# 1dayac/spades_for_blackbird

Hardware: AMD Instinct MI355X
Metric: distinct k-mers/sec (k=21, 150 bp synthetic reads, count only) (higher is better)
Workload: dtype u64

## Files before the change

### spades_for_blackbird_amd/csrc/bbk_internal.h

```cpp
#pragma once

#include <hip/hip_runtime.h>

#include <cstdint>
#include <cstdio>
#include <cstdlib>
#include <map>
#include <memory>
#include <string>
#include <type_traits>
#include <utility>
#include <vector>

#include "../../include/bbk.h"

namespace bbk {

void set_error(const char *fmt, ...);

struct Error {
    int code;
};

#define BBK_HIP(expr)                                                                          \
// ... 226 lines not shown
struct PassDesc {
    int kind;
    int word;
    int shift;
    int bits;
    unsigned nb;
};

std::vector<PassDesc> key_passes(unsigned k);

void sort_records(bbk_ctx *ctx, int W, void *keys, void *keys_tmp, uint32_t *vals, uint32_t *vals_tmp, uint64_t n,
                  const std::vector<PassDesc> &passes);
void partition_records(bbk_ctx *ctx, int W, const void *src, void *dst, const uint32_t *vsrc, uint32_t *vdst, uint64_t n,
                       const PassDesc &pd, uint64_t *h_digit_totals = nullptr);

enum ReduceOp { REDUCE_COUNT = 0, REDUCE_SUM = 1, REDUCE_OR = 2 };
uint64_t unique_records(bbk_ctx *ctx, int W, const void *keys, const uint32_t *vals, uint64_t n, void *out_keys,
                        uint32_t *out_vals, ReduceOp op, bool drop_zero);
uint64_t drop_zero_vals(bbk_ctx *ctx, int W, const void *keys, const uint32_t *vals, uint64_t n, DevBuf &out_keys,
                        DevBuf &out_vals);
uint64_t exclusive_scan_u64(bbk_ctx *ctx, const uint64_t *in, uint64_t *out, uint64_t n);
void exclusive_scan2_u64(bbk_ctx *ctx, const uint64_t *in0, uint64_t *out0, const uint64_t *in1, uint64_t *out1,
                         uint64_t n, uint64_t totals[2]);
enum { SCAN_U64 = 0, SCAN_U32_FLAGGED = 1, SCAN_SLOT_FILL = 2 };
struct ScanSrc {
    const void *p;
    uint32_t kind, stride, cap;
};
void exclusive_scan_enqueue(bbk_ctx *ctx, int narr, const ScanSrc *src, uint64_t *const *out, uint64_t n,
                            uint64_t *d_total, bool tail, std::vector<DevBuf> &keep);
struct PrefixTable;
struct PrefixIndex {
    DevBuf buf;
    unsigned bits = 0;
    bool wide = false;
    unsigned W = 0, k = 0;
    void build(bbk_ctx *ctx, const uint64_t *keys, unsigned W, unsigned k, uint64_t n);
    PrefixTable table() const;
};
size_t device_free_cached(bbk_ctx *ctx);
void *plan_staging(bbk_ctx *ctx, size_t bytes);

}

extern "C" int bbk_scan2_u64(bbk_ctx *ctx, void *d_a, void *d_b, uint64_t n, uint64_t *totals);

struct bbk_reads {
    bbk_ctx *ctx = nullptr;
    uint64_t n = 0;
    uint64_t n_words = 0;
    uint64_t bases = 0;
    const uint64_t *d_words = nullptr;
    const uint64_t *d_woff = nullptr;
    const uint32_t *d_len = nullptr;
    bbk::DevBuf own_words, own_woff, own_len;
};

struct bbk_kmerset {
    unsigned k = 0, W = 0;
    unsigned flags = 0;
    uint64_t n = 0;
    uint64_t instances = 0;
    bbk::DevBuf keys;
    bbk::DevBuf counts;
    bool has_counts = false;
    bool sorted = true;
    bool ref_order = false;
};

struct bbk_extindex {
    unsigned k = 0, W = 0;
    uint64_t n = 0;
    uint64_t instances = 0;
    bbk::DevBuf keys;
    bbk::DevBuf masks;
    bbk::PrefixIndex prefix;
};
```

### spades_for_blackbird_amd/csrc/count.hip

```cpp
#include <hip/hip_runtime.h>

#include <fcntl.h>
#include <unistd.h>

#include <algorithm>
#include <cstdio>
#include <cstring>
#include <memory>
#include <vector>

#include "bbk_internal.h"
#include "kmer_ops.h"
#include "msd.h"
#include "accum.h"

namespace bbk {

static bool msd_enabled() {
    const char *e = getenv("BBK_DISABLE_MSD");
    return !(e && e[0] == '1');
}

__global__ void k_kmers_per_read(const uint32_t *__restrict__ len, uint64_t n, uint32_t k,
                                 uint64_t *__restrict__ nk) {
    const uint64_t i = BBK_GID();
    if (i < n) {
        const uint32_t L = len[i];
        nk[i] = L >= k ? (uint64_t)(L - k + 1) : 0ull;
    }
}

template <int W, int MODE>
__global__ __launch_bounds__(256) void k_extract(const uint64_t *__restrict__ words,
                                                const uint64_t *__restrict__ woff,
                                                const uint32_t *__restrict__ len,
                                                const uint64_t *__restrict__ koff, uint64_t n_reads, int k,
                                                Key<W> *__restrict__ out, uint32_t *__restrict__ out_val) {
    const int lane = threadIdx.x & 63;
    const uint64_t wave = (BBK_GID()) >> 6;
    const uint64_t nwaves = ((uint64_t)gridDim.x * blockDim.x) >> 6;
    for (uint64_t r = wave; r < n_reads; r += nwaves) {
        const uint32_t L = len[r];
        if (L < (uint32_t)k) continue;
        const uint32_t nk = L - (uint32_t)k + 1;
        const uint64_t *rw = words + woff[r];
        const uint64_t base = koff[r];
        for (uint32_t p = lane; p < nk; p += 64) {
            const Key<W> fwd = kmer_extract<W>(rw, p, k);
            const Key<W> rc = kmer_rc<W>(fwd, k);
            const bool minimal = !kmer_less_nucl<W>(rc, fwd);
            out[base + p] = key_select<W>(minimal, fwd, rc);
            if (MODE == 1) {
// ... 125 lines not shown
    }
};

void dedup_reads(bbk_ctx *ctx, const bbk_reads *rd, unsigned k, bool with_mask, bool want_vals, DevBuf &out_keys,
                 DevBuf &out_vals, uint64_t &n_distinct, uint64_t &n_instances, BucketView *view = nullptr) {
    n_distinct = 0;
    n_instances = 0;
    if (msd_enabled()) {
        const int op1 = with_mask ? MSD_OP_OR : (want_vals ? MSD_OP_COUNT : MSD_OP_NONE);
        if (superk_dedup_reads(ctx, rd, k, op1, out_keys, out_vals, n_distinct, n_instances)) return;
        n_distinct = 0;
        n_instances = 0;
        MsdOutput a;
        a.want_view = view != nullptr;
        if (msd_sort_reduce(ctx, k, MsdRequest::reads(MSD_HASH, op1, rd, with_mask), a)) {
            n_instances = a.instances;
            n_distinct = a.n;
            if (a.view.live()) *view = std::move(a.view);
            out_keys = std::move(a.keys);
            if (op1 != MSD_OP_NONE) out_vals = std::move(a.vals);
            return;
        }
    }
    DevBuf koff((rd->n + 1) * sizeof(uint64_t));
    if (rd->n) launch_items(ctx, "k_kmers_per_read", k_kmers_per_read, rd->n, rd->d_len, rd->n, k, koff.as<uint64_t>());
    const uint64_t N = exclusive_scan_u64(ctx, koff.as<uint64_t>(), koff.as<uint64_t>(), rd->n);
    n_instances = N;
    if (N == 0) return empty_result(out_keys, &out_vals);
    BBK_REQUIRE(N < (1ull << 32), BBK_ERR_ARG,
                "batch holds %llu k-mer instances; the LSD path is limited to 2^32-1 per batch (push the reads in "
                "smaller batches)",
                (unsigned long long)N);
    LsdSort t(ctx, k, N, with_mask);
    dispatch_w(t.W, [&](auto w) {
        launch_extract<decltype(w)::value>(ctx, rd, koff.as<uint64_t>(), (int)k, t.keys.p, t.vals.as<uint32_t>(), N);
    });
    t.sort();
    n_distinct =
        t.unique(with_mask ? REDUCE_OR : REDUCE_COUNT, out_keys, (with_mask || want_vals) ? &out_vals : nullptr);
}

static uint64_t lsd_sort_unique(bbk_ctx *ctx, unsigned k, const void *d_keys, const uint32_t *d_vals, uint64_t n,
                                ReduceOp rop, DevBuf &out_keys, DevBuf &out_vals) {
    LsdSort t(ctx, k, n, d_vals != nullptr);
    t.load(d_keys, d_vals);
    t.sort();
    return t.unique(rop, out_keys, d_vals ? &out_vals : nullptr);
}

// ... 562 lines not shown
```

### spades_for_blackbird_amd/csrc/kmer_ops.h

```cpp
#pragma once

#include <hip/hip_runtime.h>
#include <stdint.h>

namespace bbk {

template <int W>
struct Key {
    uint64_t w[W];
};

template <int W>
__host__ __device__ inline bool key_eq(const Key<W> &a, const Key<W> &b) {
    bool e = true;
#pragma unroll
    for (int i = 0; i < W; ++i) e = e && (a.w[i] == b.w[i]);
    return e;
}

template <int W>
__host__ __device__ inline bool key_less_words(const Key<W> &a, const Key<W> &b) {
#pragma unroll
    for (int i = 0; i < W; ++i) {
        if (a.w[i] != b.w[i]) return a.w[i] < b.w[i];
// ... 118 lines not shown
        if (a.w[i] != b.w[i]) return rev2(a.w[i]) < rev2(b.w[i]);
    }
    return false;
}

template <int W>
__device__ inline Key<W> kmer_canon(const uint64_t *__restrict__ rw, uint32_t p, int k, uint32_t last_word, bool *minimal) {
    if constexpr (W == 1) {
        return kmer_extract_canon1(rw, p, k, last_word, minimal);
    } else {
        const Key<W> x = kmer_extract<W>(rw, p, k);
        const Key<W> r = kmer_rc<W>(x, k);
        *minimal = !kmer_less_nucl<W>(r, x);
        return key_select<W>(*minimal, x, r);
    }
}

__device__ inline uint64_t last_le(const uint64_t *__restrict__ off, uint64_t n, uint64_t x) {
    uint64_t lo = 0, hi = n - 1;
    while (lo < hi) {
        const uint64_t mid = (lo + hi + 1) >> 1;
        if (off[mid] <= x) lo = mid;
        else hi = mid - 1;
    }
    return lo;
}

template <int W>
__device__ inline Key<W> kmer_shl(const Key<W> &x, int k, uint32_t c) {
    Key<W> o;
#pragma unroll
    for (int i = 0; i < W - 1; ++i) o.w[i] = (x.w[i] >> 2) | ((x.w[i + 1] & 3ull) << 62);
    const uint32_t lastshift = (uint32_t)(((k + 31) & 31) << 1);
    o.w[W - 1] = (x.w[W - 1] >> 2) | ((uint64_t)(c & 3u) << lastshift);
    return o;
}

template <int W>
__device__ inline Key<W> kmer_shr(const Key<W> &x, int k, uint32_t c) {
    Key<W> o;
#pragma unroll
    for (int i = W - 1; i > 0; --i) o.w[i] = (x.w[i] << 2) | (x.w[i - 1] >> 62);
    o.w[0] = (x.w[0] << 2) | (uint64_t)(c & 3u);
    const int vb = 2 * k - 64 * (W - 1);
    if (vb < 64) o.w[W - 1] &= (1ull << vb) - 1ull;
    return o;
// ... 98 lines not shown
```

### spades_for_blackbird_amd/csrc/msd.h

```cpp
#pragma once

#include "bbk_internal.h"

namespace bbk {

enum { MSD_HASH = 0, MSD_KEYS = 1, MSD_REF = 2 };
enum { MSD_OP_NONE = 0, MSD_OP_COUNT = 1, MSD_OP_SUM = 2, MSD_OP_OR = 3 };

struct BucketView {
    DevBuf slots;
    DevBuf dcount;
    DevBuf off;
    DevBuf seg;
    DevBuf extra;
    uint32_t nbuckets = 0, stride = 0;
    int hb = 0;
    uint64_t D = 0, n_extra = 0;
    DevBuf keys;
    bool live() const { return slots.p != nullptr; }
    uint64_t n() const { return D + n_extra; }
    void release_slots() {
        slots.release();
        dcount.release();
        off.release();
// ... 36 lines not shown
    static MsdRequest records(int prefix, int op, const void *keys, const uint32_t *vals, uint64_t n) {
        MsdRequest r;
        r.prefix = prefix, r.op = op, r.keys = keys, r.vals = vals, r.n = n;
        return r;
    }
    static MsdRequest expand(int prefix, int op, unsigned k, const void *canon, const uint32_t *vals,
                             uint64_t n) {
        MsdRequest r = records(prefix, op, canon, vals, n);
        r.expand_k = k;
        return r;
    }
    static MsdRequest expand(int prefix, int op, unsigned k, BucketView &view) {
        MsdRequest r = expand(prefix, op, k, nullptr, nullptr, view.n());
        r.view = &view;
        return r;
    }
};

bool msd_sort_reduce(bbk_ctx *ctx, unsigned k, const MsdRequest &rq, MsdOutput &out);

bool superk_dedup_reads(bbk_ctx *ctx, const bbk_reads *rd, unsigned k, int op, DevBuf &out_keys, DevBuf &out_vals,
                        uint64_t &n_distinct, uint64_t &n_instances);

}
```

### spades_for_blackbird_amd/csrc/msd.hip

```cpp
#include <hip/hip_runtime.h>

#include <algorithm>
#include <chrono>
#include <cmath>
#include <cstdio>
#include <cstdlib>
#include <cstring>
#include <optional>
#include <type_traits>
#include <utility>
#include <vector>

#include "bbk_internal.h"
#include "kmer_ops.h"
#include "msd.h"
#include "msd.h"

#include "msd_part.h"
#include "msd_bucket.h"
#include "msd_narrow_a.h"
#include "msd_stage_b.h"

namespace bbk {

// ... 32 lines not shown
    SlotsGaveUp,
    KeySlotsGaveUp,
    NeedDense,
};

struct MsdInput {
    const bbk_reads *rd;
    const void *keys;
    const uint32_t *vals;
    uint64_t n;
    bool with_mask;
    BucketView *view = nullptr;
};

template <class F>
static void with_op(int op, F &&f) {
    switch (op) {
        case MSD_OP_NONE: f(std::integral_constant<int, MSD_OP_NONE>()); break;
        case MSD_OP_COUNT: f(std::integral_constant<int, MSD_OP_COUNT>()); break;
        case MSD_OP_SUM: f(std::integral_constant<int, MSD_OP_SUM>()); break;
        case MSD_OP_OR: f(std::integral_constant<int, MSD_OP_OR>()); break;
        default: BBK_REQUIRE(false, BBK_ERR_ARG, "bad reduce op");
    }
}

template <int W>
struct MsdRunner {
    static constexpr size_t rec = (size_t)W * 8;
    static constexpr uint32_t kPartTileK = PartCfg<W>::TILE;
    bbk_ctx *ctx;
    unsigned k;
    int dmode;
    int op;
    uint64_t strip_mask = ~0ull;
    bool assume_distinct = false;
    unsigned expand_k = 0;
    bool expand_tag = false;
    MsdKnobs knobs;
    bool slots_ok = !knobs.no_slots;
    bool kslots_ok = !knobs.no_kslots;
    bool never_decline = false;
    bool even_part = false;

    int w0bits() const { return (W == 1) ? (int)(2 * k) : 64; }

    template <class K, class... Args>
// ... 262 lines not shown
            if (auto r = first_pass()) return *r;
            if (auto r = overflow()) return *r;
            compact();
            return Outcome::Done;
        }

        bool view_level1() const {
            return W == 1 && !P.too_deep && P.kslots && R.expand_k && !ranged && !has_dst && !R.even_part && !has_val;
        }

        Outcome empty() {
            if (!has_dst) {
                out.keys.alloc(16);
                out.vals.alloc(16);
            }
            return Outcome::Done;
        }

        void count_instances() {
            N = (R.expand_k && !from_reads) ? 2 * in.n : in.n;
            if (!from_reads) return;
            const bbk_reads *rd = in.rd;
            BBK_REQUIRE(R.dmode == MSD_HASH, BBK_ERR_INTERNAL, "reads are partitioned by hash prefix only");
            DevBuf nk((rd->n + 1) * sizeof(uint64_t));
            coff.alloc((rd->n + 1) * sizeof(uint64_t));
            if (rd->n)
                R.launch_plan(k_kmers_per_read2, "k_kmers_per_read2", rd->n, rd->d_len, rd->d_woff, rd->n, R.k,
                              (uint32_t)RdCfg<W>::CH, nk.as<uint64_t>(), coff.as<uint64_t>(), ctl_at(kCtlUnordered));
            uint64_t tot[2] = {0, 0};
            exclusive_scan2_u64(ctx, nk.as<uint64_t>(), nk.as<uint64_t>(), coff.as<uint64_t>(), coff.as<uint64_t>(), rd->n,
                                tot);
            N = tot[0];
            n_chunks = tot[1];
        }

        void level1_tiles() {
            L1 = PartLevel{1, P.b1, P.nb1, R.dmode, R.w0bits(), nullptr, nullptr, sel.lo, sel.span, sel.shl, sel.mul};
            if (from_reads) {
                const bbk_reads *rd = in.rd;
                tile_read.alloc(((size_t)P.ntiles1 + 1) * sizeof(RdTile));
                tiles_h.alloc(((size_t)P.ntiles1h + 1) * sizeof(RdTile));
                if (P.ntiles1)
                    R.launch_plan(k_tile_reads, "k_tile_reads", (uint64_t)P.ntiles1 + P.ntiles1h, coff.as<uint64_t>(),
                                  rd->d_woff, rd->d_len, rd->n, (uint64_t)P.ntiles1, P.rd_tile, tile_read.as<RdTile>(),
                                  (uint64_t)P.ntiles1h, (uint32_t)kRdHistThreads, tiles_h.as<RdTile>(),
                                  (uint32_t)RdCfg<W>::CH, R.k, (uint32_t)kRdSlots, (uint32_t)kRdWords,
                                  ctl_at(kCtlUnordered));
                S = ReadSrc{rd->d_words, rd->d_woff, rd->d_len, coff.as<uint64_t>(), tile_read.as<RdTile>(), rd->n,
                            n_chunks, (int)R.k};
                Sh = S;
                Sh.tiles = tiles_h.as<RdTile>();
            }
            M1 = TileMap{nullptr, nullptr, nullptr, 1, P.Ntot, 0, 1, nullptr, (int)R.expand_k, R.expand_tag ? 1 : 0};
            if (P.slots) {
                spill_k.alloc((size_t)P.spill_cap * rec);
                if (has_val) spill_v.alloc((size_t)P.spill_cap * 4);
                use_slots(L1, P.seg_cap, P.seg_cap);
                L1.xcd_shift = P.xs;
                L1.sub_cap = P.sub_cap;
            }
        }

        void use_slots(PartLevel &L, uint32_t cap, uint32_t stride) {
            L.slot_cap = cap;
            L.slot_stride = stride;
            L.spill_keys = spill_k.p;
            L.spill_vals = spill_v.as<uint32_t>();
            L.spill_count = ctl_at(kCtlSpill);
            L.spill_cap = P.spill_cap;
            L.narrow_hb = P.narrow ? P.nw_hb : 0;
// ... 1109 lines not shown
    MsdInput in{rq.rd, rq.keys, rq.vals, rq.n, rq.with_mask};
    if (view && !view->live()) in.keys = view->keys.p;
    else in.view = view;
    if (rq.tag_bits) {
        BBK_REQUIRE(words_of(k) == 1 && rq.rd == nullptr && rq.prefix == MSD_KEYS && rq.tag_bits % 2 == 0 &&
                        2 * k + rq.tag_bits <= 64 && (rq.expand_k == 0 || rq.expand_k == k),
                    BBK_ERR_INTERNAL, "tagged sort needs 8-byte keys with %u spare bits", rq.tag_bits);
        return msd_run<1>(ctx, k + rq.tag_bits / 2, rq.prefix, rq.op, in, out, rq.assume_distinct, rq.expand_k,
                          rq.expand_k != 0, (2 * k >= 64) ? ~0ull : ((1ull << (2 * k)) - 1ull));
    }
#ifdef BBK_PHASE_PROF
    struct Dump {
        ~Dump() { dump_phases(); }
    } dump_on_exit;
#endif
    bool done = false;
    dispatch_w(words_of(k), [&](auto w) {
        done = msd_run<decltype(w)::value>(ctx, k, rq.prefix, rq.op, in, out, rq.assume_distinct, rq.expand_k);
    });
    return done;
}

}
```

### spades_for_blackbird_amd/csrc/msd_part.h

```cpp
#pragma once

namespace bbk {

#ifndef BBK_KEYS_TILE
#define BBK_KEYS_TILE 8192
#endif
#ifndef BBK_KEYS_THREADS
#define BBK_KEYS_THREADS 512
#endif
template <int W>
struct PartCfg {
    static constexpr int TILE = (W == 1) ? BBK_KEYS_TILE : (W == 2 ? 4096 : 2048);
    static constexpr int THREADS = BBK_KEYS_THREADS;
    static constexpr int ITEMS = TILE / THREADS;
};
constexpr int kRdThreads = 1024;
constexpr int kRdHistThreads = 512;
constexpr int kRdSlots = 1024;
constexpr int kRdWords = 2048;
template <int W>
struct RdCfg {
    static constexpr int CH = (W == 1) ? 8 : (W == 2 ? 4 : 2);
    static constexpr int TILE = kRdThreads * CH;
};
// ... 57 lines not shown
    int k;
};

template <class T, class I>
__device__ inline I last_le(const T *start, I n, T x) {
    I lo = 0, hi = n;
    while (hi - lo > 1) {
        const I mid = (lo + hi) >> 1;
        if (start[mid] <= x) lo = mid;
        else hi = mid;
    }
    return lo;
}

struct RdTile {
    uint64_t wbase;
    uint32_t r0;
    uint32_t nr;
    uint32_t wspan;
    uint32_t pad;
};

__global__ void k_tile_reads(const uint64_t *__restrict__ coff, const uint64_t *__restrict__ woff,
                             const uint32_t *__restrict__ len, uint64_t n_reads, uint64_t n_tiles, uint32_t tile,
                             RdTile *__restrict__ out, uint64_t n_tiles_b, uint32_t tile_b, RdTile *__restrict__ out_b,
                             uint32_t ch, uint32_t k, uint32_t max_reads, uint32_t max_words,
                             const uint32_t *__restrict__ unordered) {
    uint64_t t = BBK_GID();
    if (t >= n_tiles) {
        t -= n_tiles;
        if (t >= n_tiles_b) return;
        tile = tile_b;
        out = out_b;
    }
    const uint64_t c0 = t * (uint64_t)tile;
    const uint64_t r0 = last_le(coff, n_reads, c0), r1 = last_le(coff, n_reads, c0 + tile);
    const uint32_t p0 = (uint32_t)(c0 - coff[r0]) * ch;
    const uint64_t wbase = woff[r0] + ((p0 ? p0 - 1u : 0u) >> 5);
    const uint32_t len1 = len[r1];
    const uint64_t span1 = (c0 + tile - coff[r1]) * ch + k;
    const uint32_t lastb1 = len1 ? (uint32_t)(span1 < (uint64_t)(len1 - 1u) ? span1 : (uint64_t)(len1 - 1u)) : 0u;
    const uint64_t wend = woff[r1] + (len1 ? (lastb1 >> 5) + 1u : 0u);
    const uint64_t nr = r1 - r0 + 1;
    const bool fast = *unordered == 0 && nr <= (uint64_t)max_reads && wend >= wbase && wend - wbase <= (uint64_t)max_words;
    RdTile T;
    T.wbase = wbase;
    T.r0 = (uint32_t)r0;
    T.nr = (uint32_t)nr;
    T.wspan = fast ? (uint32_t)(wend - wbase) : 0xFFFFFFFFu;
    T.pad = 0;
    out[t] = T;
}

__global__ void k_kmers_per_read2(const uint32_t *__restrict__ len, const uint64_t *__restrict__ woff, uint64_t n,
                                  uint32_t k, uint32_t ch, uint64_t *__restrict__ nk, uint64_t *__restrict__ nch,
                                  uint32_t *__restrict__ unordered) {
    const uint64_t i = BBK_GID();
    if (i < n) {
        const uint32_t L = len[i];
        const uint64_t c = L >= k ? (uint64_t)(L - k + 1) : 0ull;
        nk[i] = c;
        nch[i] = (c + ch - 1) / ch;
        if (i + 1 < n && woff[i + 1] < woff[i] + ((L + 31u) >> 5)) *unordered = 1u;
    }
}

struct TileMap {
    const uint32_t *seg_tile_start;
    const uint32_t *seg_off;
    const uint32_t *seg_size;
    uint32_t nseg;
    uint64_t n;
    uint32_t ntiles;
    uint32_t group;
    const uint4 *desc;
    int expand_k;
    int expand_tag;
};

template <bool SEG_IN_Z>
__global__ void k_tile_desc(TileMap M, const uint32_t *__restrict__ seg_nb2, const uint32_t *__restrict__ seg_bin_start,
                            uint32_t tile_size, int sub_shift, const uint32_t *__restrict__ xstart,
                            uint4 *__restrict__ desc) {
    const uint32_t t = blockIdx.x * blockDim.x + threadIdx.x;
    if (t >= M.ntiles) return;
    const uint32_t e = last_le(M.seg_tile_start, M.nseg, t), i = t - M.seg_tile_start[e];
    const uint32_t b = M.seg_off[e] + i * tile_size;
// ... 582 lines not shown
```

### spades_for_blackbird_amd/csrc/primitives.hip

```cpp
#include <hip/hip_runtime.h>

#include <fcntl.h>
#include <unistd.h>

#include <algorithm>
#include <chrono>
#include <cstdarg>
#include <cstring>
#include <map>
#include <memory>
#include <mutex>
#include <thread>
#include <vector>

#include "arena.h"
#include "bbk_internal.h"
#include "kmer_ops.h"

namespace bbk {

static thread_local char g_err[1024] = "";
void set_error(const char *fmt, ...) {
    va_list ap;
    va_start(ap, fmt);
// ... 457 lines not shown
        if (w < wave) base += s;
        tot += s;
    }
    __syncthreads();
    *total = tot;
    return base + incl - v;
}

constexpr int kScanItems = 16;
constexpr int kScanTile = kThreads * kScanItems;

struct ScanArrs {
    ScanSrc src[2];
    uint64_t *out[2];
    uint64_t *bsum[2];
    uint64_t *total[2];
    uint64_t *tail[2];
};

__device__ inline uint64_t scan_load(const ScanSrc &s, uint64_t i) {
    if (s.kind == SCAN_U64) return reinterpret_cast<const uint64_t *>(s.p)[i];
    const uint32_t v = reinterpret_cast<const uint32_t *>(s.p)[i];
    if (s.kind == SCAN_U32_FLAGGED) return v == 0xFFFFFFFFu ? 0ull : (uint64_t)v;
    const uint32_t c = v - (uint32_t)i * s.stride;
    return c < s.cap ? c : s.cap;
}

template <int NA>
__global__ __launch_bounds__(kThreads) void k_scan_reduce(ScanArrs A, uint64_t n) {
    __shared__ uint64_t sm[NA][kWaves];
    const uint64_t base = (uint64_t)blockIdx.x * kScanTile;
#pragma unroll
    for (int a = 0; a < NA; ++a) {
        uint64_t s = 0;
#pragma unroll
        for (int i = 0; i < kScanItems; ++i) {
            const uint64_t idx = base + (uint64_t)i * kThreads + threadIdx.x;
            if (idx < n) s += scan_load(A.src[a], idx);
        }
#pragma unroll
        for (int d = 32; d >= 1; d >>= 1) s += __shfl_down(s, d, 64);
        if ((threadIdx.x & 63) == 0) sm[a][threadIdx.x >> 6] = s;
    }
    __syncthreads();
    if (threadIdx.x < NA) {
        uint64_t t = 0;
        for (int w = 0; w < kWaves; ++w) t += sm[threadIdx.x][w];
        A.bsum[threadIdx.x][blockIdx.x] = t;
    }
}

template <int NA, bool TOP>
__global__ __launch_bounds__(kThreads) void k_scan_apply(ScanArrs A, uint64_t n) {
    __shared__ uint64_t sm[NA][kWaves];
    const uint64_t base = (uint64_t)blockIdx.x * kScanTile + (uint64_t)threadIdx.x * kScanItems;
    const int lane = threadIdx.x & 63, wave = threadIdx.x >> 6;
#pragma unroll
    for (int a = 0; a < NA; ++a) {
        uint64_t v[kScanItems];
        uint64_t s = 0;
#pragma unroll
        for (int i = 0; i < kScanItems; ++i) {
            v[i] = (base + i < n) ? scan_load(A.src[a], base + i) : 0;
            s += v[i];
        }
        uint64_t incl = s;
#pragma unroll
        for (int d = 1; d < 64; d <<= 1) {
            uint64_t t = __shfl_up(incl, d, 64);
            if (lane >= d) incl += t;
        }
        if (lane == 63) sm[a][wave] = incl;
        __syncthreads();
        uint64_t wbase = 0;
        for (int w = 0; w < wave; ++w) wbase += sm[a][w];
        uint64_t run = (TOP ? 0ull : A.bsum[a][blockIdx.x]) + wbase + incl - s;
#pragma unroll
        for (int i = 0; i < kScanItems; ++i) {
            if (base + i < n) A.out[a][base + i] = run;
            run += v[i];
        }
        if (TOP && threadIdx.x == kThreads - 1) {
            *A.total[a] = run;
            if (A.tail[a]) *A.tail[a] = run;
        }
    }
}

template <int NA>
static void scan_level(bbk_ctx *ctx, ScanArrs A, uint64_t n, std::vector<DevBuf> &keep) {
    const uint64_t nb = (n + kScanTile - 1) / kScanTile;
    if (nb <= 1) {
        hipLaunchKernelGGL((k_scan_apply<NA, true>), dim3(1), dim3(kThreads), 0, ctx->stream, A, n);
        check_launch("k_scan_apply");
        return;
    }
    BBK_REQUIRE(nb < (1ull << 31), BBK_ERR_ARG, "scan of %llu items", (unsigned long long)n);
    keep.emplace_back((size_t)NA * (nb + 1) * sizeof(uint64_t));
    uint64_t *bs = keep.back().as<uint64_t>();
    ScanArrs B = A;
    for (int a = 0; a < NA; ++a) {
        A.bsum[a] = bs + (size_t)a * (nb + 1);
        B.src[a] = ScanSrc{A.bsum[a], SCAN_U64, 0u, 0u};
        B.out[a] = A.bsum[a];
    }
    hipLaunchKernelGGL((k_scan_reduce<NA>), dim3((unsigned)nb), dim3(kThreads), 0, ctx->stream, A, n);
    check_launch("k_scan_reduce");
    scan_level<NA>(ctx, B, nb, keep);
    hipLaunchKernelGGL((k_scan_apply<NA, false>), dim3((unsigned)nb), dim3(kThreads), 0, ctx->stream, A, n);
    check_launch("k_scan_apply");
}

void exclusive_scan_enqueue(bbk_ctx *ctx, int narr, const ScanSrc *src, uint64_t *const *out, uint64_t n,
                            uint64_t *d_total, bool tail, std::vector<DevBuf> &keep) {
    BBK_REQUIRE(narr == 1 || narr == 2, BBK_ERR_INTERNAL, "scan of %d arrays", narr);
    ScanArrs A{};
    for (int a = 0; a < narr; ++a) {
        A.src[a] = src[a];
        A.out[a] = out[a];
        A.total[a] = d_total + a;
        A.tail[a] = tail ? out[a] + n : nullptr;
    }
    if (narr == 1) scan_level<1>(ctx, A, n, keep);
    else scan_level<2>(ctx, A, n, keep);
}

uint64_t exclusive_scan_u64(bbk_ctx *ctx, const uint64_t *in, uint64_t *out, uint64_t n) {
    if (n == 0) return 0;
    std::vector<DevBuf> keep;
    keep.reserve(4);
    DevBuf dt(16);
    const ScanSrc src{in, SCAN_U64, 0u, 0u};
    exclusive_scan_enqueue(ctx, 1, &src, &out, n, dt.as<uint64_t>(), false, keep);
    uint64_t total = 0;
    BBK_HIP(hipMemcpyAsync(&total, dt.p, sizeof(uint64_t), hipMemcpyDeviceToHost, ctx->stream));
    stream_wait(ctx);
    return total;
}

void exclusive_scan2_u64(bbk_ctx *ctx, const uint64_t *in0, uint64_t *out0, const uint64_t *in1, uint64_t *out1,
                         uint64_t n, uint64_t totals[2]) {
    std::vector<DevBuf> keep;
    keep.reserve(4);
    DevBuf dt(16);
    const ScanSrc src[2] = {{in0, SCAN_U64, 0u, 0u}, {in1, SCAN_U64, 0u, 0u}};
    uint64_t *const out[2] = {out0, out1};
    exclusive_scan_enqueue(ctx, 2, src, out, n, dt.as<uint64_t>(), true, keep);
    BBK_HIP(hipMemcpyAsync(totals, dt.p, 2 * sizeof(uint64_t), hipMemcpyDeviceToHost, ctx->stream));
    stream_wait(ctx);
}

size_t device_free_cached(bbk_ctx *ctx) {
    uint64_t now = 0, total = 0;
    pool_stats(ctx->device, &now, &total, nullptr);
    if (now != ctx->mem_free_mapped_now || total != ctx->mem_free_mapped_total) {
        size_t fr = 0, tot = 0;
        BBK_HIP(hipMemGetInfo(&fr, &tot));
        ctx->mem_free = fr;
        ctx->mem_free_mapped_now = now;
        ctx->mem_free_mapped_total = total;
    }
    return ctx->mem_free;
}

void *plan_staging(bbk_ctx *ctx, size_t bytes) {
    if (bytes > ctx->plan_pinned_bytes) {
        if (ctx->plan_pinned) BBK_HIP(hipHostFree(ctx->plan_pinned));
        ctx->plan_pinned = nullptr;
        ctx->plan_pinned_bytes = 0;
        const size_t want = std::max<size_t>(2 * bytes, 256u << 10);
        BBK_HIP(hipHostMalloc(&ctx->plan_pinned, want, hipHostMallocDefault));
        ctx->plan_pinned_bytes = want;
// ... 696 lines not shown
```

### spades_for_blackbird_amd/csrc/superk.hip

```cpp
#include <hip/hip_runtime.h>

#include <algorithm>
#include <chrono>
#include <cmath>
#include <cstdio>
#include <cstdlib>
#include <optional>
#include <type_traits>
#include <vector>

#include "bbk_internal.h"
#include "kmer_ops.h"
#include "msd.h"

namespace bbk {

namespace {

constexpr int kSkHdrBits = 19;
constexpr int kSkHdrShift = 64 - kSkHdrBits;
constexpr int kSk1NT = 256;
constexpr int kSk2NT = 256;
constexpr int kSk2Items = 8;
constexpr int kSk2Tile = kSk2NT * kSk2Items;
// ... 92 lines not shown
        rw = r;
        wi = 0xFFFFFFFFu;
        cur = 0;
    }
    __device__ __forceinline__ uint32_t at(uint32_t p) {
        const uint32_t x = p >> 5;
        if (x != wi) {
            wi = x;
            cur = rw[x];
        }
        return (uint32_t)(cur >> ((p & 31u) << 1)) & 3u;
    }
};

__device__ inline uint64_t sk_read_at(const uint64_t *__restrict__ off, uint64_t lo, uint64_t hi, uint64_t j) {
    while (hi - lo > 1) {
        const uint64_t mid = (lo + hi) >> 1;
        if (off[mid] <= j) lo = mid;
        else hi = mid;
    }
    return lo;
}

__global__ void k_sk_segments(const uint32_t *__restrict__ len, uint64_t n, uint32_t k, uint32_t C,
                              uint64_t *__restrict__ nk, uint64_t *__restrict__ nseg) {
    const uint64_t i = (uint64_t)blockIdx.x * blockDim.x + threadIdx.x;
    if (i < n) {
        const uint32_t L = len[i];
        const uint64_t c = L >= k ? (uint64_t)(L - k + 1) : 0ull;
        nk[i] = c;
        nseg[i] = (c + C - 1) / C;
    }
}

__global__ void k_sk_tiles(const uint64_t *__restrict__ coff, uint64_t n_reads, uint64_t n_tiles, uint32_t tile,
                           uint64_t n_segs, SkTile *__restrict__ out) {
    const uint64_t t = (uint64_t)blockIdx.x * blockDim.x + threadIdx.x;
    if (t >= n_tiles) return;
    const uint64_t c0 = t * (uint64_t)tile;
    const uint64_t c1 = (c0 + tile < n_segs ? c0 + tile : n_segs) - 1;
    const uint64_t r0 = sk_read_at(coff, 0, n_reads, c0), r1 = sk_read_at(coff, 0, n_reads, c1);
    out[t] = SkTile{(uint32_t)r0, (uint32_t)(r1 - r0 + 1)};
}

template <int RW>
__device__ __forceinline__ uint64_t sk_word(const uint64_t (&rec)[RW], uint32_t wi) {
    uint64_t v = 0;
#pragma unroll
    for (int j = 0; j < RW; ++j) v = (wi == (uint32_t)j) ? rec[j] : v;
    return v;
}

template <int RW>
__device__ __forceinline__ uint32_t sk_rec_hash(const uint64_t (&rec)[RW], uint32_t m) {
    const uint32_t hdr = (uint32_t)(rec[RW - 1] >> kSkHdrShift);
    const uint32_t mp = (hdr >> 6) & 127u;
    const uint32_t wi = mp >> 5, sh = (mp & 31u) << 1;
    const uint64_t lo = sk_word<RW>(rec, wi), hi = sk_word<RW>(rec, wi + 1u);
    const uint64_t mmask = (1ull << (2u * m)) - 1ull;
    const uint64_t F = ((lo >> sh) | ((hi << 1) << (63u - sh))) & mmask;
    const uint64_t R = (~rev2(F)) >> (64u - 2u * m);
    return sk_mhash(F, R);
}

// ... 774 lines not shown
        count_segments(G.C);
        std::optional<SkPlan> plan = sk_plan<W>(ctx, kn, G, N, n_segs);
        if (!plan) return SkOutcome::NotTaken;
        L = *plan;
        setup();
        for (uint32_t pass = 0; pass < P.np; ++pass) {
            P.pass = pass;
            level1();
            if (!level2()) return declined();
            for (int attempt = 0;; ++attempt) {
                if (!dedup() || !kmer_path()) return declined();
                if (!hflags[SKF_OUT]) break;
                regrow(attempt);
            }
            done_before = cursor_now;
        }
        finish(out_keys, out_vals);
        n_instances = N;
        n_distinct = done_before;
        return SkOutcome::Done;
    }

    void count_segments(uint32_t C) {
        DevBuf nk((rd->n + 1) * sizeof(uint64_t));
        coff.alloc((rd->n + 1) * sizeof(uint64_t));
        hipLaunchKernelGGL(k_sk_segments, dim3((unsigned)((rd->n + 255) / 256)), dim3(256), 0, ctx->stream, rd->d_len, rd->n,
                           k, C, nk.as<uint64_t>(), coff.as<uint64_t>());
        check_launch("k_sk_segments");
        N = exclusive_scan_u64(ctx, nk.as<uint64_t>(), nk.as<uint64_t>(), rd->n);
        n_segs = exclusive_scan_u64(ctx, coff.as<uint64_t>(), coff.as<uint64_t>(), rd->n);
    }

    void setup() {
        BBK_HIP(hipMemcpyAsync(coff.as<uint64_t>() + rd->n, &n_segs, sizeof(uint64_t), hipMemcpyHostToDevice, ctx->stream));
        sync();
        if (kn.verbose)
            fprintf(stderr,
                    "[bbk] superk: k=%u m=%u w=%u C=%u segs=%llu est_records=%.0f passes=%u P1=%u P2=%u slot1=%u lds1=%zu fill=%.2f\n",
                    k, P.m, P.w, P.C, (unsigned long long)n_segs, L.est_total, P.np, P.P1, P.P2, P.slot1, L.sm1, L.fill);
        tiles.alloc((size_t)(L.ntiles1 + 1) * sizeof(SkTile));
        hipLaunchKernelGGL(k_sk_tiles, dim3((unsigned)((L.ntiles1 + 255) / 256)), dim3(256), 0, ctx->stream,
                           coff.as<uint64_t>(), rd->n, L.ntiles1, (uint32_t)kSk1NT, n_segs, tiles.as<SkTile>());
        check_launch("k_sk_tiles");
        S = SkReads{rd->d_words, rd->d_woff, rd->d_len, coff.as<uint64_t>(), tiles.as<SkTile>(), rd->n, n_segs};
        if (kn.verbose) {
            sync();
            t_setup = since();
        }
        buf1.alloc((size_t)P.P1 * P.slot1 * rec_bytes);
        cur1.alloc((size_t)P.P1 * 8 * 4 + 16);
        boff.alloc((size_t)(L.nbuckets + 1) * 8 + 16);
        cur2.alloc((size_t)L.nbuckets * 8 + 16);
        dflags.alloc(64);
        dcursor.alloc(16);
        fail_list.alloc((size_t)kSkdFailCap * 4);
        fail2_list.alloc((size_t)kSkdFailCap * 4);
        fb_total.alloc(16);
        spill.alloc((size_t)P.spill_cap * rec_bytes + 16);
        BBK_HIP(hipMemsetAsync(dflags.p, 0, 64, ctx->stream));
        BBK_HIP(hipMemsetAsync(dcursor.p, 0, 16, ctx->stream));
        out_cap = L.out_cap;
        okeys.alloc(out_cap * key_bytes + 16);
        if (has_vals) ovals.alloc(out_cap * 4 + 16);
        if (kn.verbose) {
            sync();
            t_alloc = since();
// ... 194 lines not shown
        ctx->add_stat("stat_superk_declined", 1);
        ctx->superk_dup = 0;
        return SkOutcome::Declined;
    }
};

}

bool superk_dedup_reads(bbk_ctx *ctx, const bbk_reads *rd, unsigned k, int op, DevBuf &out_keys, DevBuf &out_vals,
                        uint64_t &n_distinct, uint64_t &n_instances) {
    const SuperkKnobs kn;
    if (kn.no_superk) return false;
    auto run = [&](auto w) {
        SuperkRun<decltype(w)::value> R(ctx, rd, k, op, kn);
        return R.run(out_keys, out_vals, n_distinct, n_instances) == SkOutcome::Done;
    };
    const unsigned W = words_of(k);
    if (W == 2) return run(std::integral_constant<int, 2>());
    if (W == 3) return run(std::integral_constant<int, 3>());
    if (W == 4) return run(std::integral_constant<int, 4>());
    return false;
}

}
```

Baseline: 29.97 billion.

## Fuse per-read k-mer/segment counting into scan loads with shared ReadPlan

Replaces the separate per-read count kernels (k_kmers_per_read, k_kmers_per_read2, k_sk_segments) with a scan input kind that computes k-mer and chunk counts directly from read lengths, and folds the woff ordering check into the scan. The k-mer count scan no longer writes an output array, and the superk path drops a host-to-device copy and a sync. Tile-to-read lookup switches from plain binary search to an interpolation guess plus galloping search. It also adds exported read-plan entry points. Together these are meant to cut kernel launches, intermediate buffers and memory traffic in the planning phase, at the cost of more logic inside the scan loads.

```diff
diff --git a/spades_for_blackbird_amd/csrc/bbk_internal.h b/spades_for_blackbird_amd/csrc/bbk_internal.h
--- a/spades_for_blackbird_amd/csrc/bbk_internal.h
+++ b/spades_for_blackbird_amd/csrc/bbk_internal.h
@@ -272,10 +272,12 @@
 uint64_t exclusive_scan_u64(bbk_ctx *ctx, const uint64_t *in, uint64_t *out, uint64_t n);
 void exclusive_scan2_u64(bbk_ctx *ctx, const uint64_t *in0, uint64_t *out0, const uint64_t *in1, uint64_t *out1,
                          uint64_t n, uint64_t totals[2]);
-enum { SCAN_U64 = 0, SCAN_U32_FLAGGED = 1, SCAN_SLOT_FILL = 2 };
+enum { SCAN_U64 = 0, SCAN_U32_FLAGGED = 1, SCAN_SLOT_FILL = 2, SCAN_READ_UNITS = 3 };
 struct ScanSrc {
     const void *p;
     uint32_t kind, stride, cap;
+    const uint64_t *woff = nullptr;
+    uint32_t *unordered = nullptr;
 };
 void exclusive_scan_enqueue(bbk_ctx *ctx, int narr, const ScanSrc *src, uint64_t *const *out, uint64_t n,
                             uint64_t *d_total, bool tail, std::vector<DevBuf> &keep);
@@ -294,6 +296,11 @@
 }
 
 extern "C" int bbk_scan2_u64(bbk_ctx *ctx, void *d_a, void *d_b, uint64_t n, uint64_t *totals);
+struct bbk_reads;
+extern "C" int bbk_read_plan_geometry(unsigned k, uint32_t *out);
+extern "C" int bbk_read_plan(bbk_ctx *ctx, const bbk_reads *rd, unsigned k, unsigned C, unsigned tile, int superk,
+                             uint64_t *coff, uint64_t *totals, uint32_t *unordered, void *tiles, uint64_t tile_cap,
+                             uint64_t *n_tiles);
 
 struct bbk_reads {
     bbk_ctx *ctx = nullptr;
@@ -305,6 +312,16 @@
     const uint32_t *d_len = nullptr;
     bbk::DevBuf own_words, own_woff, own_len;
 };
+
+namespace bbk {
+
+struct ReadPlan {
+    DevBuf coff;
+    uint64_t kmers = 0, units = 0;
+    void run(bbk_ctx *ctx, const bbk_reads *rd, unsigned k, unsigned C, uint32_t *d_unordered);
+};
+
+}
 
 struct bbk_kmerset {
     unsigned k = 0, W = 0;
diff --git a/spades_for_blackbird_amd/csrc/count.hip b/spades_for_blackbird_amd/csrc/count.hip
--- a/spades_for_blackbird_amd/csrc/count.hip
+++ b/spades_for_blackbird_amd/csrc/count.hip
@@ -19,15 +19,6 @@
 static bool msd_enabled() {
     const char *e = getenv("BBK_DISABLE_MSD");
     return !(e && e[0] == '1');
-}
-
-__global__ void k_kmers_per_read(const uint32_t *__restrict__ len, uint64_t n, uint32_t k,
-                                 uint64_t *__restrict__ nk) {
-    const uint64_t i = BBK_GID();
-    if (i < n) {
-        const uint32_t L = len[i];
-        nk[i] = L >= k ? (uint64_t)(L - k + 1) : 0ull;
-    }
 }
 
 template <int W, int MODE>
@@ -199,9 +190,10 @@
             return;
         }
     }
-    DevBuf koff((rd->n + 1) * sizeof(uint64_t));
-    if (rd->n) launch_items(ctx, "k_kmers_per_read", k_kmers_per_read, rd->n, rd->d_len, rd->n, k, koff.as<uint64_t>());
-    const uint64_t N = exclusive_scan_u64(ctx, koff.as<uint64_t>(), koff.as<uint64_t>(), rd->n);
+    ReadPlan rp;
+    rp.run(ctx, rd, k, 1u, nullptr);
+    const DevBuf &koff = rp.coff;
+    const uint64_t N = rp.kmers;
     n_instances = N;
     if (N == 0) return empty_result(out_keys, &out_vals);
     BBK_REQUIRE(N < (1ull << 32), BBK_ERR_ARG,
diff --git a/spades_for_blackbird_amd/csrc/kmer_ops.h b/spades_for_blackbird_amd/csrc/kmer_ops.h
--- a/spades_for_blackbird_amd/csrc/kmer_ops.h
+++ b/spades_for_blackbird_amd/csrc/kmer_ops.h
@@ -164,6 +164,41 @@
         const uint64_t mid = (lo + hi + 1) >> 1;
         if (off[mid] <= x) lo = mid;
         else hi = mid - 1;
+    }
+    return lo;
+}
+
+constexpr int kReadGallop = 8;
+__device__ inline uint64_t read_of_unit(const uint64_t *__restrict__ coff, uint64_t n, uint64_t units, uint64_t c) {
+    if (c >= units) return n - 1;
+    uint64_t g = (uint64_t)((double)c * (double)n / (double)units);
+    if (g > n - 1) g = n - 1;
+    uint64_t lo = 0, hi = n;
+    if (coff[g] <= c) {
+        lo = g;
+        uint64_t d = 1;
+        for (int s = 0; s < kReadGallop && lo + d < n; ++s, d <<= 1) {
+            if (coff[lo + d] > c) {
+                hi = lo + d;
+                break;
+            }
+            lo += d;
+        }
+    } else {
+        hi = g;
+        uint64_t d = 1;
+        for (int s = 0; s < kReadGallop && hi > d; ++s, d <<= 1) {
+            if (coff[hi - d] <= c) {
+                lo = hi - d;
+                break;
+            }
+            hi -= d;
+        }
+    }
+    while (hi - lo > 1) {
+        const uint64_t mid = (lo + hi) >> 1;
+        if (coff[mid] <= c) lo = mid;
+        else hi = mid;
     }
     return lo;
 }
diff --git a/spades_for_blackbird_amd/csrc/msd.h b/spades_for_blackbird_amd/csrc/msd.h
--- a/spades_for_blackbird_amd/csrc/msd.h
+++ b/spades_for_blackbird_amd/csrc/msd.h
@@ -82,4 +82,9 @@
 bool superk_dedup_reads(bbk_ctx *ctx, const bbk_reads *rd, unsigned k, int op, DevBuf &out_keys, DevBuf &out_vals,
                         uint64_t &n_distinct, uint64_t &n_instances);
 
+uint32_t superk_segment_len(unsigned k);
+uint32_t superk_tile_segments();
+void superk_plan_tiles(bbk_ctx *ctx, const uint64_t *coff, uint64_t n_reads, uint64_t n_segs, uint32_t tile,
+                       uint64_t n_tiles, DevBuf &tiles);
+
 }
diff --git a/spades_for_blackbird_amd/csrc/msd.hip b/spades_for_blackbird_amd/csrc/msd.hip
--- a/spades_for_blackbird_amd/csrc/msd.hip
+++ b/spades_for_blackbird_amd/csrc/msd.hip
@@ -78,6 +78,14 @@
         case MSD_OP_OR: f(std::integral_constant<int, MSD_OP_OR>()); break;
         default: BBK_REQUIRE(false, BBK_ERR_ARG, "bad reduce op");
     }
+}
+
+static void launch_tile_reads(bbk_ctx *ctx, const bbk_reads *rd, const uint64_t *coff, uint64_t n_chunks, uint64_t n_a,
+                              uint32_t tile_a, RdTile *out_a, uint64_t n_b, uint32_t tile_b, RdTile *out_b, uint32_t ch,
+                              uint32_t k, const uint32_t *unordered) {
+    if (n_a + n_b == 0) return;
+    launch_items(ctx, "k_tile_reads", k_tile_reads, n_a + n_b, coff, rd->d_woff, rd->d_len, rd->n, n_chunks, n_a, tile_a,
+                 out_a, n_b, tile_b, out_b, ch, k, (uint32_t)kRdSlots, (uint32_t)kRdWords, unordered);
 }
 
 template <int W>
@@ -386,30 +394,24 @@
             if (!from_reads) return;
             const bbk_reads *rd = in.rd;
             BBK_REQUIRE(R.dmode == MSD_HASH, BBK_ERR_INTERNAL, "reads are partitioned by hash prefix only");
-            DevBuf nk((rd->n + 1) * sizeof(uint64_t));
-            coff.alloc((rd->n + 1) * sizeof(uint64_t));
-            if (rd->n)
-                R.launch_plan(k_kmers_per_read2, "k_kmers_per_read2", rd->n, rd->d_len, rd->d_woff, rd->n, R.k,
-                              (uint32_t)RdCfg<W>::CH, nk.as<uint64_t>(), coff.as<uint64_t>(), ctl_at(kCtlUnordered));
-            uint64_t tot[2] = {0, 0};
-            exclusive_scan2_u64(ctx, nk.as<uint64_t>(), nk.as<uint64_t>(), coff.as<uint64_t>(), coff.as<uint64_t>(), rd->n,
-                                tot);
-            N = tot[0];
-            n_chunks = tot[1];
+            ReadPlan rp;
+            rp.run(ctx, rd, R.k, (unsigned)RdCfg<W>::CH, ctl_at(kCtlUnordered));
+            coff = std::move(rp.coff);
+            N = rp.kmers;
+            n_chunks = rp.units;
         }
 
         void level1_tiles() {
             L1 = PartLevel{1, P.b1, P.nb1, R.dmode, R.w0bits(), nullptr, nullptr, sel.lo, sel.span, sel.shl, sel.mul};
             if (from_reads) {
                 const bbk_reads *rd = in.rd;
+                const uint64_t nth = P.slots ? 0 : P.ntiles1h;
                 tile_read.alloc(((size_t)P.ntiles1 + 1) * sizeof(RdTile));
-                tiles_h.alloc(((size_t)P.ntiles1h + 1) * sizeof(RdTile));
+                tiles_h.alloc(((size_t)nth + 1) * sizeof(RdTile));
                 if (P.ntiles1)
-                    R.launch_plan(k_tile_reads, "k_tile_reads", (uint64_t)P.ntiles1 + P.ntiles1h, coff.as<uint64_t>(),
-                                  rd->d_woff, rd->d_len, rd->n, (uint64_t)P.ntiles1, P.rd_tile, tile_read.as<RdTile>(),
-                                  (uint64_t)P.ntiles1h, (uint32_t)kRdHistThreads, tiles_h.as<RdTile>(),
-                                  (uint32_t)RdCfg<W>::CH, R.k, (uint32_t)kRdSlots, (uint32_t)kRdWords,
-                                  ctl_at(kCtlUnordered));
+                    launch_tile_reads(ctx, rd, coff.as<uint64_t>(), n_chunks, P.ntiles1, P.rd_tile, tile_read.as<RdTile>(),
+                                      nth, (uint32_t)kRdHistThreads, tiles_h.as<RdTile>(), (uint32_t)RdCfg<W>::CH, R.k,
+                                      ctl_at(kCtlUnordered));
                 S = ReadSrc{rd->d_words, rd->d_woff, rd->d_len, coff.as<uint64_t>(), tile_read.as<RdTile>(), rd->n,
                             n_chunks, (int)R.k};
                 Sh = S;
@@ -1565,3 +1567,49 @@
 }
 
 }
+
+extern "C" int bbk_read_plan_geometry(unsigned k, uint32_t *out) {
+    return bbk::guarded([&] {
+        BBK_REQUIRE(out && k >= 1, BBK_ERR_ARG, "bbk_read_plan_geometry: bad argument");
+        uint32_t ch = 0;
+        bbk::dispatch_w(bbk::words_of(k), [&](auto w) { ch = (uint32_t)bbk::RdCfg<decltype(w)::value>::CH; });
+        const uint32_t g[10] = {ch, (uint32_t)bbk::kRdThreads, (uint32_t)bbk::kRdHistThreads,
+                                (uint32_t)bbk::NwCfg<false>::CHUNKS, (uint32_t)bbk::NwCfg<true>::CHUNKS,
+                                bbk::superk_segment_len(k), bbk::superk_tile_segments(), (uint32_t)bbk::kRdSlots,
+                                (uint32_t)bbk::kRdWords, 0u};
+        for (int i = 0; i < 10; ++i) out[i] = g[i];
+    });
+}
+
+extern "C" int bbk_read_plan(bbk_ctx *ctx, const bbk_reads *rd, unsigned k, unsigned C, unsigned tile, int superk,
+                             uint64_t *coff, uint64_t *totals, uint32_t *unordered, void *tiles, uint64_t tile_cap,
+                             uint64_t *n_tiles) {
+    using namespace bbk;
+    return guarded([&] {
+        BBK_REQUIRE(ctx && rd && coff && totals && unordered && tiles && n_tiles && k >= 1 && C >= 1 && tile >= 1, BBK_ERR_ARG,
+                    "bbk_read_plan: bad argument");
+        BBK_HIP(hipSetDevice(ctx->device));
+        DevBuf flag(16), td;
+        BBK_HIP(hipMemsetAsync(flag.p, 0, 16, ctx->stream));
+        ReadPlan rp;
+        rp.run(ctx, rd, k, C, flag.as<uint32_t>());
+        const uint64_t nt = (rp.units + tile - 1) / tile;
+        BBK_REQUIRE(nt <= tile_cap, BBK_ERR_ARG, "bbk_read_plan: %llu tiles, room for %llu", (unsigned long long)nt,
+                    (unsigned long long)tile_cap);
+        size_t tile_bytes = sizeof(RdTile);
+        if (superk) {
+            superk_plan_tiles(ctx, rp.coff.as<uint64_t>(), rd->n, rp.units, tile, nt, td);
+            tile_bytes = 8;
+        } else {
+            td.alloc((size_t)(nt + 1) * sizeof(RdTile));
+            launch_tile_reads(ctx, rd, rp.coff.as<uint64_t>(), rp.units, nt, (uint32_t)tile, td.as<RdTile>(), 0, (uint32_t)tile,
+                              td.as<RdTile>(), (uint32_t)C, (uint32_t)k, flag.as<uint32_t>());
+        }
+        totals[0] = rp.kmers;
+        totals[1] = rp.units;
+        *n_tiles = nt;
+        d2h_sync(ctx, coff, rp.coff.p, (size_t)(rd->n + 1) * sizeof(uint64_t));
+        d2h_sync(ctx, unordered, flag.p, sizeof(uint32_t));
+        if (nt) d2h_sync(ctx, tiles, td.p, (size_t)nt * tile_bytes);
+    });
+}
diff --git a/spades_for_blackbird_amd/csrc/msd_part.h b/spades_for_blackbird_amd/csrc/msd_part.h
--- a/spades_for_blackbird_amd/csrc/msd_part.h
+++ b/spades_for_blackbird_amd/csrc/msd_part.h
@@ -103,9 +103,9 @@
 };
 
 __global__ void k_tile_reads(const uint64_t *__restrict__ coff, const uint64_t *__restrict__ woff,
-                             const uint32_t *__restrict__ len, uint64_t n_reads, uint64_t n_tiles, uint32_t tile,
-                             RdTile *__restrict__ out, uint64_t n_tiles_b, uint32_t tile_b, RdTile *__restrict__ out_b,
-                             uint32_t ch, uint32_t k, uint32_t max_reads, uint32_t max_words,
+                             const uint32_t *__restrict__ len, uint64_t n_reads, uint64_t n_chunks, uint64_t n_tiles,
+                             uint32_t tile, RdTile *__restrict__ out, uint64_t n_tiles_b, uint32_t tile_b,
+                             RdTile *__restrict__ out_b, uint32_t ch, uint32_t k, uint32_t max_reads, uint32_t max_words,
                              const uint32_t *__restrict__ unordered) {
     uint64_t t = BBK_GID();
     if (t >= n_tiles) {
@@ -115,7 +115,7 @@
         out = out_b;
     }
     const uint64_t c0 = t * (uint64_t)tile;
-    const uint64_t r0 = last_le(coff, n_reads, c0), r1 = last_le(coff, n_reads, c0 + tile);
+    const uint64_t r0 = read_of_unit(coff, n_reads, n_chunks, c0), r1 = read_of_unit(coff, n_reads, n_chunks, c0 + tile);
     const uint32_t p0 = (uint32_t)(c0 - coff[r0]) * ch;
     const uint64_t wbase = woff[r0] + ((p0 ? p0 - 1u : 0u) >> 5);
     const uint32_t len1 = len[r1];
@@ -131,19 +131,6 @@
     T.wspan = fast ? (uint32_t)(wend - wbase) : 0xFFFFFFFFu;
     T.pad = 0;
     out[t] = T;
-}
-
-__global__ void k_kmers_per_read2(const uint32_t *__restrict__ len, const uint64_t *__restrict__ woff, uint64_t n,
-                                  uint32_t k, uint32_t ch, uint64_t *__restrict__ nk, uint64_t *__restrict__ nch,
-                                  uint32_t *__restrict__ unordered) {
-    const uint64_t i = BBK_GID();
-    if (i < n) {
-        const uint32_t L = len[i];
-        const uint64_t c = L >= k ? (uint64_t)(L - k + 1) : 0ull;
-        nk[i] = c;
-        nch[i] = (c + ch - 1) / ch;
-        if (i + 1 < n && woff[i + 1] < woff[i] + ((L + 31u) >> 5)) *unordered = 1u;
-    }
 }
 
 struct TileMap {
diff --git a/spades_for_blackbird_amd/csrc/primitives.hip b/spades_for_blackbird_amd/csrc/primitives.hip
--- a/spades_for_blackbird_amd/csrc/primitives.hip
+++ b/spades_for_blackbird_amd/csrc/primitives.hip
@@ -503,8 +503,19 @@
     if (s.kind == SCAN_U64) return reinterpret_cast<const uint64_t *>(s.p)[i];
     const uint32_t v = reinterpret_cast<const uint32_t *>(s.p)[i];
     if (s.kind == SCAN_U32_FLAGGED) return v == 0xFFFFFFFFu ? 0ull : (uint64_t)v;
+    if (s.kind == SCAN_READ_UNITS) {
+        const uint32_t c = v >= s.stride ? v - s.stride + 1u : 0u;
+        if (c == 0u) return 0ull;
+        const uint32_t q = (s.cap & (s.cap - 1u)) ? (c - 1u) / s.cap : (c - 1u) >> (__ffs(s.cap) - 1);
+        return (uint64_t)q + 1ull;
+    }
     const uint32_t c = v - (uint32_t)i * s.stride;
     return c < s.cap ? c : s.cap;
+}
+
+__device__ inline bool scan_out_of_order(const ScanSrc &s, uint64_t i, uint64_t n) {
+    const uint32_t L = reinterpret_cast<const uint32_t *>(s.p)[i];
+    return i + 1 < n && s.woff[i + 1] < s.woff[i] + ((L + 31u) >> 5);
 }
 
 template <int NA>
@@ -514,11 +525,17 @@
 #pragma unroll
     for (int a = 0; a < NA; ++a) {
         uint64_t s = 0;
+        const bool check = A.src[a].kind == SCAN_READ_UNITS && A.src[a].woff;
+        bool bad = false;
 #pragma unroll
         for (int i = 0; i < kScanItems; ++i) {
             const uint64_t idx = base + (uint64_t)i * kThreads + threadIdx.x;
-            if (idx < n) s += scan_load(A.src[a], idx);
-        }
+            if (idx < n) {
+                s += scan_load(A.src[a], idx);
+                if (check) bad |= scan_out_of_order(A.src[a], idx, n);
+            }
+        }
+        if (bad) *A.src[a].unordered = 1u;
 #pragma unroll
         for (int d = 32; d >= 1; d >>= 1) s += __shfl_down(s, d, 64);
         if ((threadIdx.x & 63) == 0) sm[a][threadIdx.x >> 6] = s;
@@ -538,13 +555,19 @@
     const int lane = threadIdx.x & 63, wave = threadIdx.x >> 6;
 #pragma unroll
     for (int a = 0; a < NA; ++a) {
+        const bool store = A.out[a] != nullptr;
+        if (!TOP && !store) continue;
         uint64_t v[kScanItems];
         uint64_t s = 0;
+        const bool check = TOP && A.src[a].kind == SCAN_READ_UNITS && A.src[a].woff;
+        bool bad = false;
 #pragma unroll
         for (int i = 0; i < kScanItems; ++i) {
             v[i] = (base + i < n) ? scan_load(A.src[a], base + i) : 0;
             s += v[i];
-        }
+            if (check && base + i < n) bad |= scan_out_of_order(A.src[a], base + i, n);
+        }
+        if (bad) *A.src[a].unordered = 1u;
         uint64_t incl = s;
 #pragma unroll
         for (int d = 1; d < 64; d <<= 1) {
@@ -558,7 +581,7 @@
         uint64_t run = (TOP ? 0ull : A.bsum[a][blockIdx.x]) + wbase + incl - s;
 #pragma unroll
         for (int i = 0; i < kScanItems; ++i) {
-            if (base + i < n) A.out[a][base + i] = run;
+            if (store && base + i < n) A.out[a][base + i] = run;
             run += v[i];
         }
         if (TOP && threadIdx.x == kThreads - 1) {
@@ -600,7 +623,7 @@
         A.src[a] = src[a];
         A.out[a] = out[a];
         A.total[a] = d_total + a;
-        A.tail[a] = tail ? out[a] + n : nullptr;
+        A.tail[a] = (tail && out[a]) ? out[a] + n : nullptr;
     }
     if (narr == 1) scan_level<1>(ctx, A, n, keep);
     else scan_level<2>(ctx, A, n, keep);
@@ -629,6 +652,25 @@
     exclusive_scan_enqueue(ctx, 2, src, out, n, dt.as<uint64_t>(), true, keep);
     BBK_HIP(hipMemcpyAsync(totals, dt.p, 2 * sizeof(uint64_t), hipMemcpyDeviceToHost, ctx->stream));
     stream_wait(ctx);
+}
+
+void ReadPlan::run(bbk_ctx *ctx, const bbk_reads *rd, unsigned k, unsigned C, uint32_t *d_unordered) {
+    BBK_REQUIRE(k >= 1 && C >= 1, BBK_ERR_INTERNAL, "read plan: k = %u, C = %u", k, C);
+    const uint64_t n = rd->n;
+    coff.alloc((n + 1) * sizeof(uint64_t));
+    std::vector<DevBuf> keep;
+    keep.reserve(4);
+    DevBuf dt(16);
+    const ScanSrc src[2] = {{rd->d_len, SCAN_READ_UNITS, k, 1u},
+                            {rd->d_len, SCAN_READ_UNITS, k, C, d_unordered ? rd->d_woff : nullptr, d_unordered}};
+    uint64_t *const out[2] = {nullptr, coff.as<uint64_t>()};
+    const int first = C == 1 ? 1 : 0;
+    exclusive_scan_enqueue(ctx, 2 - first, src + first, out + first, n, dt.as<uint64_t>(), true, keep);
+    uint64_t tot[2] = {0, 0};
+    BBK_HIP(hipMemcpyAsync(tot, dt.p, (2 - first) * sizeof(uint64_t), hipMemcpyDeviceToHost, ctx->stream));
+    stream_wait(ctx);
+    kmers = tot[0];
+    units = tot[1 - first];
 }
 
 size_t device_free_cached(bbk_ctx *ctx) {
diff --git a/spades_for_blackbird_amd/csrc/superk.hip b/spades_for_blackbird_amd/csrc/superk.hip
--- a/spades_for_blackbird_amd/csrc/superk.hip
+++ b/spades_for_blackbird_amd/csrc/superk.hip
@@ -138,24 +138,13 @@
     return lo;
 }
 
-__global__ void k_sk_segments(const uint32_t *__restrict__ len, uint64_t n, uint32_t k, uint32_t C,
-                              uint64_t *__restrict__ nk, uint64_t *__restrict__ nseg) {
-    const uint64_t i = (uint64_t)blockIdx.x * blockDim.x + threadIdx.x;
-    if (i < n) {
-        const uint32_t L = len[i];
-        const uint64_t c = L >= k ? (uint64_t)(L - k + 1) : 0ull;
-        nk[i] = c;
-        nseg[i] = (c + C - 1) / C;
-    }
-}
-
 __global__ void k_sk_tiles(const uint64_t *__restrict__ coff, uint64_t n_reads, uint64_t n_tiles, uint32_t tile,
                            uint64_t n_segs, SkTile *__restrict__ out) {
-    const uint64_t t = (uint64_t)blockIdx.x * blockDim.x + threadIdx.x;
+    const uint64_t t = BBK_GID();
     if (t >= n_tiles) return;
     const uint64_t c0 = t * (uint64_t)tile;
     const uint64_t c1 = (c0 + tile < n_segs ? c0 + tile : n_segs) - 1;
-    const uint64_t r0 = sk_read_at(coff, 0, n_reads, c0), r1 = sk_read_at(coff, 0, n_reads, c1);
+    const uint64_t r0 = read_of_unit(coff, n_reads, n_segs, c0), r1 = read_of_unit(coff, n_reads, n_segs, c1);
     out[t] = SkTile{(uint32_t)r0, (uint32_t)(r1 - r0 + 1)};
 }
 
@@ -976,26 +965,19 @@
     }
 
     void count_segments(uint32_t C) {
-        DevBuf nk((rd->n + 1) * sizeof(uint64_t));
-        coff.alloc((rd->n + 1) * sizeof(uint64_t));
-        hipLaunchKernelGGL(k_sk_segments, dim3((unsigned)((rd->n + 255) / 256)), dim3(256), 0, ctx->stream, rd->d_len, rd->n,
-                           k, C, nk.as<uint64_t>(), coff.as<uint64_t>());
-        check_launch("k_sk_segments");
-        N = exclusive_scan_u64(ctx, nk.as<uint64_t>(), nk.as<uint64_t>(), rd->n);
-        n_segs = exclusive_scan_u64(ctx, coff.as<uint64_t>(), coff.as<uint64_t>(), rd->n);
+        ReadPlan rp;
+        rp.run(ctx, rd, k, C, nullptr);
+        coff = std::move(rp.coff);
+        N = rp.kmers;
+        n_segs = rp.units;
     }
 
     void setup() {
-        BBK_HIP(hipMemcpyAsync(coff.as<uint64_t>() + rd->n, &n_segs, sizeof(uint64_t), hipMemcpyHostToDevice, ctx->stream));
-        sync();
         if (kn.verbose)
             fprintf(stderr,
                     "[bbk] superk: k=%u m=%u w=%u C=%u segs=%llu est_records=%.0f passes=%u P1=%u P2=%u slot1=%u lds1=%zu fill=%.2f\n",
                     k, P.m, P.w, P.C, (unsigned long long)n_segs, L.est_total, P.np, P.P1, P.P2, P.slot1, L.sm1, L.fill);
-        tiles.alloc((size_t)(L.ntiles1 + 1) * sizeof(SkTile));
-        hipLaunchKernelGGL(k_sk_tiles, dim3((unsigned)((L.ntiles1 + 255) / 256)), dim3(256), 0, ctx->stream,
-                           coff.as<uint64_t>(), rd->n, L.ntiles1, (uint32_t)kSk1NT, n_segs, tiles.as<SkTile>());
-        check_launch("k_sk_tiles");
+        superk_plan_tiles(ctx, coff.as<uint64_t>(), rd->n, n_segs, (uint32_t)kSk1NT, L.ntiles1, tiles);
         S = SkReads{rd->d_words, rd->d_woff, rd->d_len, coff.as<uint64_t>(), tiles.as<SkTile>(), rd->n, n_segs};
         if (kn.verbose) {
             sync();
@@ -1236,4 +1218,22 @@
     return false;
 }
 
-}
+uint32_t superk_segment_len(unsigned k) {
+    const SuperkKnobs kn;
+    switch (words_of(k)) {
+        case 2: return sk_geometry<2>(k, kn).C;
+        case 3: return sk_geometry<3>(k, kn).C;
+        case 4: return sk_geometry<4>(k, kn).C;
+        default: return 0;
+    }
+}
+
+uint32_t superk_tile_segments() { return (uint32_t)kSk1NT; }
+
+void superk_plan_tiles(bbk_ctx *ctx, const uint64_t *coff, uint64_t n_reads, uint64_t n_segs, uint32_t tile,
+                       uint64_t n_tiles, DevBuf &tiles) {
+    tiles.alloc((size_t)(n_tiles + 1) * sizeof(SkTile));
+    if (n_tiles) launch_items(ctx, "k_sk_tiles", k_sk_tiles, n_tiles, coff, n_reads, n_tiles, tile, n_segs, tiles.as<SkTile>());
+}
+
+}
```

Result: faster. 30.67 billion, median of 6 (+2.3%).
